# goroda/c3sc

Hardware: AMD Instinct MI355X
Metric: Bellman-sweep nodes/sec (7D car rank-10) (higher is better)
Workload: dtype f64

## Files before the change

c3sc_amd/csrc/c3sc_hip.hip:

```cpp
#include <hip/hip_runtime.h>

#include <algorithm>
#include <cmath>
#include <cstdio>
#include <cstdlib>
#include <cstring>
#include <string>
#include <vector>

#include "../../include/c3sc_hip.h"
#include "fiber_partition.hpp"
#include "kernel_chain_walk.hpp"
#include "kernel_common.hpp"
#include "kernel_rollout.hpp"
#include "kernel_rollout_ode.hpp"
#include "model_tables.hpp"
#include "registry.hpp"

namespace c3sc {

std::vector<KernelEntry> &kernel_registry()
{
    static std::vector<KernelEntry> reg;
    return reg;
}

__global__ void k_pad_core(const double *__restrict__ src, double *__restrict__ dst, int N, int r0, int r1, int RP,
                           int kind )
{
    const int per = (kind == 1) ? RP * RP : RP;
    const long total = (long)N * per;
    for (long e = (long)blockIdx.x * blockDim.x + threadIdx.x; e < total; e += (long)gridDim.x * blockDim.x) {
        const int j = (int)(e / per), w = (int)(e - (long)j * per);
        int a, b;
        if (kind == 0) { a = 0; b = w; }
        else if (kind == 2) { a = w; b = 0; }
        else { a = w % RP; b = w / RP; }
        double v = 0.0;
        if (a < r0 && b < r1) v = src[(size_t)j * r0 * r1 + a + (size_t)b * r0];
// ... 21 lines not shown
        const long total = (long)J.nodes[jb] * n2 * RP;
        for (long e = (long)blockIdx.x * blockDim.x + threadIdx.x; e < total; e += (long)gridDim.x * blockDim.x) {
            const long row = e / RP;
            const int c = (int)(e - row * RP), a = (int)(row / n2), b = (int)(row - (long)a * n2);
            const double *vec = left ? core + (size_t)a * RP : core2 + (size_t)b * RP;
            const double *mat = left ? core2 + (size_t)b * RP * RP + (size_t)c * RP : core + (size_t)a * RP * RP + c;
            const int ms = left ? 1 : RP;
            double t = 0.0;
            for (int s = 0; s < RP; s++) t = fma(vec[s], mat[(size_t)s * ms], t);
            img[e] = t;
        }
        return;
    }
    const long total = (long)J.nodes[jb] * stride;
    for (long e = (long)blockIdx.x * blockDim.x + threadIdx.x; e < total; e += (long)gridDim.x * blockDim.x) {
        const int j = (int)(e / stride), w = (int)(e - (long)j * stride);
        img[e] = (w < per) ? core[(size_t)j * per + w] : 0.0;
    }
}

struct Tab3Jobs {
    long tab2[2], core[2], dst[2];
    int n3[2], npairs[2];
};
__global__ void k_pair_tab3(double *__restrict__ arena, const Tab3Jobs J, int RP)
{
    const int sd = blockIdx.y;
    const bool left = sd == 0;
    const double *tab2 = arena + J.tab2[sd], *core = arena + J.core[sd];
    double *dst = arena + J.dst[sd];
    const long np = J.npairs[sd], total = (long)J.n3[sd] * np * RP;
    for (long e = (long)blockIdx.x * blockDim.x + threadIdx.x; e < total; e += (long)gridDim.x * blockDim.x) {
        const long row = e / RP;
        const int c = (int)(e - row * RP);
        const long i3 = row / np, pair = row - i3 * np;
        const double *vec = tab2 + pair * RP;
        const double *mat = left ? core + i3 * RP * RP + (long)c * RP : core + i3 * RP * RP + c;
        const int ms = left ? 1 : RP;
        double t = 0.0;
        for (int s = 0; s < RP; s++) t = fma(vec[s], mat[(long)s * ms], t);
        dst[e] = t;
    }
}

__global__ void k_quad_aux(const double *__restrict__ core, double *__restrict__ coreT, double *__restrict__ aop, int N, int RP)
{
    const int C = RP / 4, MB = (C + 3) / 4;
    const int per_t = RP * RP, per_a = 2 * MB * C * 64;
    const long total = (long)N * (per_t + per_a);
    for (long e = (long)blockIdx.x * blockDim.x + threadIdx.x; e < total; e += (long)gridDim.x * blockDim.x) {
        const int j = (int)(e / (per_t + per_a)), w = (int)(e - (long)j * (per_t + per_a));
// ... 753 lines not shown
        double *dst[MAXD];
        for (int m = 0; m < d; m++) dst[m] = buf.data() + (offs[(size_t)s * MAXD + m] - (long)c->static_doubles);
        pad_cores_host(d, c->ngrid, rps[s], ranks + (size_t)s * (d + 1), cores + (size_t)s * d, dst);
    }
    HIPCHK(c, hipSetDevice(c->device));
    if (c->hz_stack) HIPCHK(c, hipFree(c->hz_stack));
    c->hz_stack = nullptr;
    c->hz_nstack = 0;
    HIPCHK(c, hipMalloc((void **)&c->hz_stack, off * sizeof(double)));
    HIPCHK(c, hipMemcpy(c->hz_stack + c->static_doubles, buf.data(), buf.size() * sizeof(double), hipMemcpyHostToDevice));
    c->hz_stack_static = c->static_doubles;
    c->hz_rp.swap(rps);
    c->hz_core_off.swap(offs);
    c->hz_nstack = nstack;
    return C3SC_OK;
}

int c3sc_hip_upload_value_device(c3sc_hip_ctx *c, const size_t *ranks, const double *const *d_cores, void *stream)
{
    size_t cd = 0;
    int rc = prepare_value(c, ranks, &cd);
    if (rc != C3SC_OK) return rc;
    const int d = c->d, rp = c->rp;
    for (int m = 0; m < d; m++) {
        const int kind = (m == 0) ? 0 : (m == d - 1 ? 2 : 1);
        const long total = (long)c->ngrid[m] * (kind == 1 ? rp * rp : rp);
        const int grid = (int)std::min<long>((total + 255) / 256, 1024);
        hipLaunchKernelGGL(k_pad_core, dim3(grid), dim3(256), 0, (hipStream_t)stream, d_cores[m], c->arena + c->core_off[m],
                           c->ngrid[m], (int)ranks[m], (int)ranks[m + 1], rp, kind);
    }
    HIPCHK(c, hipGetLastError());
    rc = make_quad_aux(c, stream);
    if (rc != C3SC_OK) return rc;
    c->have_value = true;
    return C3SC_OK;
}

static int fill_args(c3sc_hip_ctx *c, int k, size_t F, KArgs &A, bool need_model)
{
    if (!c) return C3SC_ERR_ARG;
    if (c->d == 0 || !c->have_boundary || !c->have_value) return fail(c, C3SC_ERR_ARG, "launch: grid, boundary and value must be set");
    if (need_model && (!c->have_mca || c->model == 0 || c->ncand == 0))
        return fail(c, C3SC_ERR_ARG, "launch: mca, model and controls must be set");
    if (k < 0 || k >= c->d) return fail(c, C3SC_ERR_ARG, "launch: dim_vary out of range");
    HIPCHK(c, hipSetDevice(c->device));
    if (c->static_dirty) {
        if (static_layout(c) != c->static_doubles)
            return fail(c, C3SC_ERR_ARG, "launch: static data changed size after upload_value; upload the value again");
        int rc = upload_static(c);
        if (rc != C3SC_OK) return rc;
    }
    std::memset(&A, 0, sizeof(A));
    A.d = c->d;
// ... 52 lines not shown
    A.memo_keys = c->memo.keys; A.memo_vals = c->memo.vals; A.memo_capmask = c->memo.capmask; A.memo_epoch_bits = c->memo.epoch_bits;
    A.memo_shift = c->memo.shift; A.memo_counters = c->memo.counters; A.memo_mode = c->memo.mode;
    for (int m = 0; m < c->d; m++) A.memo_stride[m] = c->memo.stride[m];
    c->memo.applied = true;
}

static hipError_t ctx_launch(const c3sc_hip_ctx *c, const KernelEntry &e, const KArgs &A, LaunchIO io)
{
    io.form = c->switches;
    return launch_entry(e, A, io);
}

static int launch_one(c3sc_hip_ctx *c, const KernelEntry *e, const KArgs &A, const LaunchIO &io, const char *unsupported = nullptr)
{
    c->last_kernel = e->name;
    g_launches++;
    c->status_cache_valid = false;
    const hipError_t he = ctx_launch(c, *e, A, io);
    if (he == hipErrorNotSupported && unsupported) return fail(c, C3SC_ERR_UNSUPPORTED, unsupported);
    HIPCHK(c, he);
    return C3SC_OK;
}

constexpr long FIBER_PARTITION_MIN = 524288;
static long fiber_partition_min()
{
    const char *e = getenv("C3SC_FIBER_PARTITION");
    if (!e || !*e) return FIBER_PARTITION_MIN;
    const long v = atol(e);
    return v > 0 ? v : -1;
}

static long fiber_group_floor()
{
    const char *e = getenv("C3SC_FIBER_GROUP");
    if (!e || !*e) return FPART_MIN_PER_BIN;
    const long v = atol(e);
    return v > 0 ? v : -1;
}

static bool partitions(const KernelEntry *e, const KArgs &A)
{
    if (e->variant != C3SC_VARIANT_FIBER_PAIR || e->rtc || A.ncand > 64) return false;
    bool faces = false;
    for (int m = 0; m < A.d; m++) faces = faces || (m != A.k && A.bctype[m] == C3SC_ABSORB);
    const long fmin = fiber_partition_min();
    return faces && fmin >= 0 && A.F >= fmin && A.F <= 0x40000000L;
}

static bool runs_tab3(const c3sc_hip_ctx *c, const KernelEntry *e, const KArgs &A)
{
    if (!c->tab3L_off || fpp_table3_optout(A.d, e->rp, A.k) || !partitions(e, A)) return false;
    const char *env = getenv("C3SC_PAIR_TABLE3");
    return !(env && *env && atol(env) == 0);
}

static int ensure_tab3(c3sc_hip_ctx *c, hipStream_t st)
{
    if (!c->tab3_stale) {
        if (st != c->tab3_stream) HIPCHK(c, hipStreamWaitEvent(st, c->tab3_ev, 0));
        return C3SC_OK;
    }
    const int d = c->d, rp = c->rp;
    if (!c->tab3_ev) HIPCHK(c, hipEventCreateWithFlags(&c->tab3_ev, hipEventDisableTiming));
    Tab3Jobs J;
    J.tab2[0] = c->tabL_off; J.core[0] = c->core_off[2]; J.dst[0] = c->tab3L_off;
    J.n3[0] = c->ngrid[2]; J.npairs[0] = c->ngrid[0] * c->ngrid[1];
    J.tab2[1] = c->tabR_off; J.core[1] = c->core_off[d - 3]; J.dst[1] = c->tab3R_off;
    J.n3[1] = c->ngrid[d - 3]; J.npairs[1] = c->ngrid[d - 2] * c->ngrid[d - 1];
    const long total = std::max((long)J.n3[0] * J.npairs[0], (long)J.n3[1] * J.npairs[1]) * rp;
    hipLaunchKernelGGL(k_pair_tab3, dim3((unsigned)std::min<long>((total + 255) / 256, 4096), 2), dim3(256), 0, st, c->arena, J, rp);
    HIPCHK(c, hipGetLastError());
    HIPCHK(c, hipEventRecord(c->tab3_ev, st));
    c->tab3_stream = st;
    c->tab3_stale = false;
    return C3SC_OK;
}

static int partition_fibers(c3sc_hip_ctx *c, const KernelEntry *e, const KArgs &A, LaunchIO &io, int slot, int &launched)
{
    io.perm = nullptr;
    io.nlive = nullptr;
    launched = 0;
    if (!partitions(e, A)) return C3SC_OK;
    PartArgs P;
    P.d = A.d;
    P.k = A.k;
    P.F = A.F;
    for (int m = 0; m < MAXD; m++) { P.ngrid[m] = A.ngrid[m]; P.bctype[m] = A.bctype[m]; }
    fpart_plan(P, fpp_group_levels(A.d, e->rp, A.k), fiber_group_floor());
    const size_t need = fpart_bytes(A.F, P.nbins);
    if (need > c->part_bytes[slot]) {
        if (c->part[slot]) HIPCHK(c, hipFree(c->part[slot]));
        c->part[slot] = nullptr;
        c->part_bytes[slot] = 0;
        c->part_last[slot] = {};
        HIPCHK(c, hipMalloc(&c->part[slot], need));
        c->part_bytes[slot] = need;
    }
    const PartScratch ps = fpart_carve(c->part[slot], A.F, P.nbins);
    c->part_last[slot] = {ps.perm, ps.nlive, A.F, io.stream};
    HIPCHK(c, fpart_launch(P, io.idx, ps, io.stream));
    launched = 3;
    io.perm = ps.perm;
    io.nlive = ps.nlive;
    return C3SC_OK;
}

static int launch_bellman(c3sc_hip_ctx *c, int k, size_t F, const int32_t *d_idx, const int32_t *d_policy, double *d_out,
                          int32_t *d_uidx, int32_t *d_absorbed, void *stream, int part_slot = 0)
{
    KArgs A;
    int rc = fill_args(c, k, F, A, true);
    if (rc != C3SC_OK) return rc;
    int variant = c->variant;
    for (const FormRow &r : FORM_ROWS) {
        if (!(ctx_form(c) & r.bit)) continue;
        rc = check_form_model(c, "bellman_fibers", r.bit);
        if (rc != C3SC_OK) return rc;
        if (variant != C3SC_VARIANT_AUTO && variant != C3SC_VARIANT_FIBER_PER_WAVE)
            return fails(c, C3SC_ERR_UNSUPPORTED, "bellman_fibers: " + verb(r, "runs", "run") + " on the fiber-per-wave kernel only (the pair and quad variants have no " +
                                                      r.kind + " form)");
        variant = C3SC_VARIANT_FIBER_PER_WAVE;
    }
    if (F == 0) return C3SC_OK;
// ... 938 lines not shown
```

c3sc_amd/csrc/fiber_partition.hpp:

```cpp
#pragma once
#include <hip/hip_runtime.h>

#include "kernel_common.hpp"

namespace c3sc {

constexpr int FPART_THREADS = 256, FPART_PER_THREAD = 4, FPART_BLOCK = FPART_THREADS * FPART_PER_THREAD;
static_assert(FPART_BLOCK == 1024, "the scatter packs (bin, position in the block) into one word with 10 position bits");
constexpr int FPART_BIN_PER_THREAD = 8, FPART_MAX_BINS = FPART_THREADS * FPART_BIN_PER_THREAD;
constexpr long FPART_MIN_PER_BIN = 128;
constexpr int FPART_SCAN_BINS = 16;

struct PartArgs {
    int d, k;
    long F;
    int ngrid[MAXD];
    int bctype[MAXD];
    int kmaj = -1, kmin = -1;
    int nmin = 1;
    int nbins = 2;
};

constexpr void fpart_plan(PartArgs &P, KeyLevels kl, long floor)
{
    P.kmaj = P.kmin = -1;
    P.nmin = 1;
    P.nbins = 2;
    if (floor < 0 || kl.n < 1) return;
    const long nmaj = P.ngrid[kl.major];
    if (nmaj + 1 > FPART_MAX_BINS || P.F < floor * nmaj) return;
    P.kmaj = kl.major;
    P.nbins = (int)nmaj + 1;
    if (kl.n < 2) return;
    const long nkeys = nmaj * P.ngrid[kl.minor];
    if (nkeys + 1 > FPART_MAX_BINS || P.F < floor * nkeys) return;
    P.kmin = kl.minor;
    P.nmin = P.ngrid[kl.minor];
    P.nbins = (int)nkeys + 1;
}

struct PartScratch {
    int32_t *perm = nullptr;
    int32_t *counts = nullptr;
    int32_t *totals = nullptr;
    int32_t *nlive = nullptr;
    uint16_t *bins = nullptr;
};

__host__ __device__ constexpr size_t fpart_align(size_t b) { return (b + 255) & ~(size_t)255; }
constexpr long fpart_blocks(long F) { return (F + FPART_BLOCK - 1) / FPART_BLOCK; }
struct PartOffsets {
    size_t perm, counts, totals, nlive, bins, end;
};
constexpr PartOffsets fpart_offsets(long F, int nbins)
{
    PartOffsets o{};
    o.perm = 0;
    o.counts = o.perm + fpart_align((size_t)F * 4);
    o.totals = o.counts + fpart_align((size_t)fpart_blocks(F) * nbins * 4);
    o.nlive = o.totals + fpart_align((size_t)nbins * 4);
    o.bins = o.nlive + fpart_align(4);
    o.end = o.bins + fpart_align((size_t)F * 2);
    return o;
}
constexpr size_t fpart_bytes(long F, int nbins) { return fpart_offsets(F, nbins).end; }
inline PartScratch fpart_carve(void *base, long F, int nbins)
{
    const PartOffsets o = fpart_offsets(F, nbins);
    PartScratch s;
    char *p = (char *)base;
    s.perm = (int32_t *)(p + o.perm);
    s.counts = (int32_t *)(p + o.counts);
    s.totals = (int32_t *)(p + o.totals);
    s.nlive = (int32_t *)(p + o.nlive);
    s.bins = (uint16_t *)(p + o.bins);
    return s;
}

__device__ inline bool fiber_dead(const PartArgs &P, const int32_t *__restrict__ idx, long f)
{
    bool dead = false;
    for (int m = 0; m < P.d; m++) {
        if (m == P.k) continue;
        int lo, hi;
        dead = fixed_neighbors(idx[f * P.d + m], P.ngrid[m], P.bctype[m], lo, hi) || dead;
    }
    return dead;
}

__device__ inline int fpart_block_scan(int v, int &total)
{
    __shared__ int wsum[FPART_THREADS / 64];
    const int lane = threadIdx.x & 63, w = threadIdx.x >> 6;
    int inc = v;
#pragma unroll
    for (int o = 1; o < 64; o <<= 1) {
        const int t = __shfl_up(inc, o, 64);
        if (lane >= o) inc += t;
    }
    __syncthreads();
    if (lane == 63) wsum[w] = inc;
    __syncthreads();
    int before = 0;
    total = 0;
#pragma unroll
    for (int q = 0; q < FPART_THREADS / 64; q++) {
        if (q < w) before += wsum[q];
        total += wsum[q];
    }
    return before + inc - v;
}

__global__ void __launch_bounds__(FPART_THREADS) k_fpart_count(const PartArgs P, const int32_t *__restrict__ idx, uint16_t *__restrict__ bins,
                                                               int32_t *__restrict__ counts)
{
    __shared__ int hist[FPART_MAX_BINS];
    for (int b = threadIdx.x; b < P.nbins; b += FPART_THREADS) hist[b] = 0;
    __syncthreads();
    const long f0 = (long)blockIdx.x * FPART_BLOCK + threadIdx.x;
#pragma unroll
    for (int i = 0; i < FPART_PER_THREAD; i++) {
        const long f = f0 + (long)i * FPART_THREADS;
        if (f < P.F) {
            int bin = P.nbins - 1;
            if (!fiber_dead(P, idx, f)) {
                bin = P.kmaj >= 0 ? idx[f * P.d + P.kmaj] : 0;
                if (P.kmin >= 0) bin = bin * P.nmin + idx[f * P.d + P.kmin];
                bin = min(max(bin, 0), P.nbins - 2);
            }
            bins[f] = (uint16_t)bin;
            atomicAdd(&hist[bin], 1);
        }
    }
    __syncthreads();
    int32_t *row = counts + (size_t)blockIdx.x * P.nbins;
    for (int b = threadIdx.x; b < P.nbins; b += FPART_THREADS) row[b] = hist[b];
}

constexpr int FPART_SCAN_THREADS = 1024, FPART_SCAN_CHUNK = 8;
__global__ void __launch_bounds__(FPART_SCAN_THREADS) k_fpart_scan(int32_t *__restrict__ counts, long nblocks, int nbins, int32_t *__restrict__ totals)
{
    constexpr int NS = FPART_SCAN_THREADS / FPART_SCAN_BINS;
    __shared__ int part[NS][FPART_SCAN_BINS];
    const int c = threadIdx.x % FPART_SCAN_BINS, s = threadIdx.x / FPART_SCAN_BINS;
    const int bin = blockIdx.x * FPART_SCAN_BINS + c;
    const bool on = bin < nbins;
    const long per = (nblocks + NS - 1) / NS, b0 = s * per < nblocks ? s * per : nblocks, b1 = b0 + per < nblocks ? b0 + per : nblocks;
    int sum = 0;
    if (on)
        for (long b = b0; b < b1; b += FPART_SCAN_CHUNK) {
            int v[FPART_SCAN_CHUNK];
#pragma unroll
            for (int q = 0; q < FPART_SCAN_CHUNK; q++) v[q] = b + q < b1 ? counts[(size_t)(b + q) * nbins + bin] : 0;
#pragma unroll
            for (int q = 0; q < FPART_SCAN_CHUNK; q++) sum += v[q];
        }
    part[s][c] = sum;
    __syncthreads();
    int run = 0, total = 0;
    for (int q = 0; q < NS; q++) {
        const int v = part[q][c];
        if (q < s) run += v;
        total += v;
    }
    if (on) {
        for (long b = b0; b < b1; b += FPART_SCAN_CHUNK) {
            int v[FPART_SCAN_CHUNK];
#pragma unroll
            for (int q = 0; q < FPART_SCAN_CHUNK; q++) v[q] = b + q < b1 ? counts[(size_t)(b + q) * nbins + bin] : 0;
#pragma unroll
            for (int q = 0; q < FPART_SCAN_CHUNK; q++) {
                if (b + q < b1) counts[(size_t)(b + q) * nbins + bin] = run;
                run += v[q];
            }
        }
        if (s == 0) totals[bin] = total;
    }
}

__global__ void __launch_bounds__(FPART_THREADS) k_fpart_scatter(long F, int nbins, const uint16_t *__restrict__ bins, const int32_t *__restrict__ counts,
                                                                 const int32_t *__restrict__ totals, int32_t *__restrict__ nlive,
                                                                 int32_t *__restrict__ perm)
{
    __shared__ int base[FPART_MAX_BINS];
    __shared__ int start[FPART_MAX_BINS];
    __shared__ unsigned srt[FPART_BLOCK];
    const int tid = threadIdx.x;
    {
        int v[FPART_BIN_PER_THREAD], sum = 0;
#pragma unroll
        for (int i = 0; i < FPART_BIN_PER_THREAD; i++) {
            const int b = tid * FPART_BIN_PER_THREAD + i;
            v[i] = b < nbins ? totals[b] : 0;
            sum += v[i];
        }
        int total;
        int ex = fpart_block_scan(sum, total);
#pragma unroll
        for (int i = 0; i < FPART_BIN_PER_THREAD; i++) {
            base[tid * FPART_BIN_PER_THREAD + i] = ex;
            ex += v[i];
        }
    }
    const long fb = (long)blockIdx.x * FPART_BLOCK;
    if (nbins == 2) {
        if (blockIdx.x == 0 && tid == 0) *nlive = base[1];
        bool dead[FPART_PER_THREAD];
        int live = 0;
#pragma unroll
        for (int i = 0; i < FPART_PER_THREAD; i++) {
            const long f = fb + tid * FPART_PER_THREAD + i;
            dead[i] = f < F ? bins[f] != 0 : true;
            live += dead[i] ? 0 : 1;
        }
        int total;
        const int ex = fpart_block_scan(live, total);
        const int32_t *row = counts + (size_t)blockIdx.x * 2;
        long lpos = (long)row[0] + ex, dpos = (long)base[1] + row[1] + (tid * FPART_PER_THREAD - ex);
#pragma unroll
        for (int i = 0; i < FPART_PER_THREAD; i++) {
            const long f = fb + tid * FPART_PER_THREAD + i;
            if (f < F) {
                if (dead[i]) perm[dpos++] = (int32_t)f;
                else perm[lpos++] = (int32_t)f;
            }
        }
        return;
    }
#pragma unroll
    for (int i = 0; i < FPART_PER_THREAD; i++) {
        const int p = tid * FPART_PER_THREAD + i;
        srt[p] = fb + p < F ? ((unsigned)bins[fb + p] << 10) | (unsigned)p : 0xffffffffu;
    }
    for (int k = 2; k <= FPART_BLOCK; k <<= 1)
        for (int j = k >> 1; j > 0; j >>= 1) {
            __syncthreads();
#pragma unroll
            for (int e = tid; e < FPART_BLOCK / 2; e += FPART_THREADS) {
                const int lo = ((e & ~(j - 1)) << 1) | (e & (j - 1)), hi = lo | j;
                const unsigned a = srt[lo], b = srt[hi];
                const bool up = (lo & k) == 0;
                if ((a > b) == up) {
                    srt[lo] = b;
                    srt[hi] = a;
                }
            }
        }
    __syncthreads();
    if (blockIdx.x == 0 && tid == 0) *nlive = base[nbins - 1];
    unsigned w[FPART_PER_THREAD];
#pragma unroll
    for (int i = 0; i < FPART_PER_THREAD; i++) {
        const int s = tid * FPART_PER_THREAD + i;
        w[i] = srt[s];
        if (w[i] != 0xffffffffu && (s == 0 || (srt[s - 1] >> 10) != (w[i] >> 10))) start[w[i] >> 10] = s;
    }
    __syncthreads();
    const int32_t *row = counts + (size_t)blockIdx.x * nbins;
#pragma unroll
    for (int i = 0; i < FPART_PER_THREAD; i++) {
        if (w[i] != 0xffffffffu) {
            const int s = tid * FPART_PER_THREAD + i, bin = (int)(w[i] >> 10);
            perm[(long)base[bin] + row[bin] + (s - start[bin])] = (int32_t)(fb + (w[i] & 1023u));
        }
    }
}

inline hipError_t fpart_launch(const PartArgs &P, const int32_t *idx, const PartScratch &s, hipStream_t stream)
{
    const long nb = fpart_blocks(P.F);
    hipLaunchKernelGGL(k_fpart_count, dim3((unsigned)nb), dim3(FPART_THREADS), 0, stream, P, idx, s.bins, s.counts);
    hipLaunchKernelGGL(k_fpart_scan, dim3((unsigned)((P.nbins + FPART_SCAN_BINS - 1) / FPART_SCAN_BINS)), dim3(FPART_SCAN_THREADS), 0, stream, s.counts, nb,
                       P.nbins, s.totals);
    hipLaunchKernelGGL(k_fpart_scatter, dim3((unsigned)nb), dim3(FPART_THREADS), 0, stream, P.F, P.nbins, (const uint16_t *)s.bins,
                       (const int32_t *)s.counts, (const int32_t *)s.totals, s.nlive, s.perm);
    return hipGetLastError();
}

}
```

c3sc_amd/csrc/kernel_common.hpp:

```cpp
#pragma once
#ifdef __HIPCC_RTC__
#include "rtc_prelude.hpp"
#else
#include <type_traits>
#include <hip/hip_runtime.h>
#include <stdint.h>
#endif

#include "../../include/c3sc_hip.h"

#ifdef C3SC_STAMPS
#define C3SC_STAMPS_ON 1
#else
#define C3SC_STAMPS_ON 0
#endif

namespace c3sc {

constexpr int MAXD = C3SC_MAX_DIM;

struct KArgs {
    int d, k, N, ncand;
    long F;
    int ngrid[MAXD];
// ... 63 lines not shown
    if (nl > 0 && nr > 0) return {2, k - 1, k + 1};
    if (nl > 0) return {nl > 1 ? 2 : 1, k - 1, nl > 1 ? k - 2 : -1};
    if (nr > 0) return {nr > 1 ? 2 : 1, k + 1, nr > 1 ? k + 2 : -1};
    return {0, -1, -1};
}
#ifndef FPP_DIRECT_MAXD
#define FPP_DIRECT_MAXD 3
#endif
#ifndef FPP_EDGE_TABLES
#define FPP_EDGE_TABLES 1
#endif
#ifndef FPP_GROUP_FOLD
#define FPP_GROUP_FOLD 1
#endif
__host__ __device__ constexpr bool fpp_group_fold_optout(int d, int rp, int k) { return d == 7 && rp == 10 && k == 1; }
__host__ __device__ constexpr bool fpp_table3_registered(int d, int rp) { return FPP_EDGE_TABLES && d == 7 && rp == 10; }
__host__ __device__ constexpr bool pair_tab3_reserved(int d, const int *ngrid, int rp)
{
    return d >= 6 && fpp_table3_registered(d, rp) &&
           pair_tab3_doubles(ngrid[0], ngrid[1], ngrid[2], rp) * (long)sizeof(double) <= PAIR_TAB3_MAX_BYTES &&
           pair_tab3_doubles(ngrid[d - 3], ngrid[d - 2], ngrid[d - 1], rp) * (long)sizeof(double) <= PAIR_TAB3_MAX_BYTES;
}
__host__ __device__ constexpr bool fpp_table3_optout(int d, int rp, int k) { return d == 7 && rp == 10 && k >= 2; }
__host__ __device__ constexpr KeyLevels fpp_group_levels(int d, int rp, int k)
{
    const bool direct = d <= FPP_DIRECT_MAXD && rp <= 8;
    if (!FPP_GROUP_FOLD || direct || fpp_group_fold_optout(d, rp, k)) return {0, -1, -1};
    return fpp_key_levels(d, k, FPP_EDGE_TABLES && d >= 4);
}

__device__ inline int game_list_to_pair(const KArgs &A, int p)
{
    return A.game_order == C3SC_GAME_MAXMIN ? (p % A.game_gsz) * A.game_ngrp + p / A.game_gsz : p;
}
__device__ inline int game_pair_to_list(const KArgs &A, int i)
{
    return A.game_order == C3SC_GAME_MAXMIN ? (i % A.game_ngrp) * A.game_gsz + i / A.game_ngrp : i;
}

template <class M>
struct GameOf : M {
    static constexpr bool GAME = true;
};
template <class Model>
constexpr bool model_game()
{
// ... 1019 lines not shown
```

Baseline: 34.55 billion.

## Add rank-based fiber partition, batch core padding, trim unused table side

Replaces the per-block bitonic sort in the fiber partition scatter with a rank-based scheme that records each fiber's slot during counting, and pads count rows to cache-line strides. Core padding becomes a single batched launch across all dimensions. The pair table-3 precompute now builds only the sides that some sweep dimension reads, and the partition threshold is lowered so more sweeps use partitioning. This adds a new scratch array and more complex counting, and the lower threshold may apply partitioning overhead to smaller sweeps.

```diff
diff --git a/c3sc_amd/csrc/c3sc_hip.hip b/c3sc_amd/csrc/c3sc_hip.hip
--- a/c3sc_amd/csrc/c3sc_hip.hip
+++ b/c3sc_amd/csrc/c3sc_hip.hip
@@ -10,11 +10,13 @@
 
 #include "../../include/c3sc_hip.h"
 #include "fiber_partition.hpp"
+#include "fiber_partition_sort.hpp"
 #include "kernel_chain_walk.hpp"
 #include "kernel_common.hpp"
 #include "kernel_rollout.hpp"
 #include "kernel_rollout_ode.hpp"
 #include "model_tables.hpp"
+#include "pad_cores.hpp"
 #include "registry.hpp"
 
 namespace c3sc {
@@ -82,11 +84,12 @@
 struct Tab3Jobs {
     long tab2[2], core[2], dst[2];
     int n3[2], npairs[2];
+    int left[2];
 };
 __global__ void k_pair_tab3(double *__restrict__ arena, const Tab3Jobs J, int RP)
 {
     const int sd = blockIdx.y;
-    const bool left = sd == 0;
+    const bool left = J.left[sd] != 0;
     const double *tab2 = arena + J.tab2[sd], *core = arena + J.core[sd];
     double *dst = arena + J.dst[sd];
     const long np = J.npairs[sd], total = (long)J.n3[sd] * np * RP;
@@ -886,13 +889,18 @@
     int rc = prepare_value(c, ranks, &cd);
     if (rc != C3SC_OK) return rc;
     const int d = c->d, rp = c->rp;
+    PadJobs J{};
+    J.d = d;
+    long maxtotal = 1;
     for (int m = 0; m < d; m++) {
-        const int kind = (m == 0) ? 0 : (m == d - 1 ? 2 : 1);
-        const long total = (long)c->ngrid[m] * (kind == 1 ? rp * rp : rp);
-        const int grid = (int)std::min<long>((total + 255) / 256, 1024);
-        hipLaunchKernelGGL(k_pad_core, dim3(grid), dim3(256), 0, (hipStream_t)stream, d_cores[m], c->arena + c->core_off[m],
-                           c->ngrid[m], (int)ranks[m], (int)ranks[m + 1], rp, kind);
-    }
+        J.src[m] = d_cores[m];
+        J.dst[m] = c->core_off[m];
+        J.N[m] = c->ngrid[m];
+        J.r0[m] = (int)ranks[m];
+        J.r1[m] = (int)ranks[m + 1];
+        maxtotal = std::max(maxtotal, (long)c->ngrid[m] * ((m == 0 || m == d - 1) ? rp : rp * rp));
+    }
+    HIPCHK(c, pad_cores_launch(c->arena, J, rp, (unsigned)std::min<long>((maxtotal + 255) / 256, 1024), (hipStream_t)stream));
     HIPCHK(c, hipGetLastError());
     rc = make_quad_aux(c, stream);
     if (rc != C3SC_OK) return rc;
@@ -991,7 +999,7 @@
     return C3SC_OK;
 }
 
-constexpr long FIBER_PARTITION_MIN = 524288;
+constexpr long FIBER_PARTITION_MIN = 262144;
 static long fiber_partition_min()
 {
     const char *e = getenv("C3SC_FIBER_PARTITION");
@@ -1006,6 +1014,12 @@
     if (!e || !*e) return FPART_MIN_PER_BIN;
     const long v = atol(e);
     return v > 0 ? v : -1;
+}
+
+static bool fiber_rank()
+{
+    const char *e = getenv("C3SC_FIBER_RANK");
+    return !(e && *e && atol(e) == 0);
 }
 
 static bool partitions(const KernelEntry *e, const KArgs &A)
@@ -1032,14 +1046,28 @@
     }
     const int d = c->d, rp = c->rp;
     if (!c->tab3_ev) HIPCHK(c, hipEventCreateWithFlags(&c->tab3_ev, hipEventDisableTiming));
-    Tab3Jobs J;
-    J.tab2[0] = c->tabL_off; J.core[0] = c->core_off[2]; J.dst[0] = c->tab3L_off;
-    J.n3[0] = c->ngrid[2]; J.npairs[0] = c->ngrid[0] * c->ngrid[1];
-    J.tab2[1] = c->tabR_off; J.core[1] = c->core_off[d - 3]; J.dst[1] = c->tab3R_off;
-    J.n3[1] = c->ngrid[d - 3]; J.npairs[1] = c->ngrid[d - 2] * c->ngrid[d - 1];
-    const long total = std::max((long)J.n3[0] * J.npairs[0], (long)J.n3[1] * J.npairs[1]) * rp;
-    hipLaunchKernelGGL(k_pair_tab3, dim3((unsigned)std::min<long>((total + 255) / 256, 4096), 2), dim3(256), 0, st, c->arena, J, rp);
-    HIPCHK(c, hipGetLastError());
+    Tab3Jobs J{};
+    const Tab3Sides sides = fpp_table3_sides(d, rp);
+    int n = 0;
+    long total = 0;
+    if (sides.left) {
+        J.left[n] = 1;
+        J.tab2[n] = c->tabL_off; J.core[n] = c->core_off[2]; J.dst[n] = c->tab3L_off;
+        J.n3[n] = c->ngrid[2]; J.npairs[n] = c->ngrid[0] * c->ngrid[1];
+        total = std::max(total, (long)J.n3[n] * J.npairs[n] * rp);
+        n++;
+    }
+    if (sides.right) {
+        J.left[n] = 0;
+        J.tab2[n] = c->tabR_off; J.core[n] = c->core_off[d - 3]; J.dst[n] = c->tab3R_off;
+        J.n3[n] = c->ngrid[d - 3]; J.npairs[n] = c->ngrid[d - 2] * c->ngrid[d - 1];
+        total = std::max(total, (long)J.n3[n] * J.npairs[n] * rp);
+        n++;
+    }
+    if (n > 0) {
+        hipLaunchKernelGGL(k_pair_tab3, dim3((unsigned)std::min<long>((total + 255) / 256, 4096), (unsigned)n), dim3(256), 0, st, c->arena, J, rp);
+        HIPCHK(c, hipGetLastError());
+    }
     HIPCHK(c, hipEventRecord(c->tab3_ev, st));
     c->tab3_stream = st;
     c->tab3_stale = false;
@@ -1069,7 +1097,7 @@
     }
     const PartScratch ps = fpart_carve(c->part[slot], A.F, P.nbins);
     c->part_last[slot] = {ps.perm, ps.nlive, A.F, io.stream};
-    HIPCHK(c, fpart_launch(P, io.idx, ps, io.stream));
+    HIPCHK(c, fiber_rank() ? fpart_launch(P, io.idx, ps, io.stream) : fpart_launch_sorting(P, io.idx, ps, io.stream));
     launched = 3;
     io.perm = ps.perm;
     io.nlive = ps.nlive;
diff --git a/c3sc_amd/csrc/fiber_partition.hpp b/c3sc_amd/csrc/fiber_partition.hpp
--- a/c3sc_amd/csrc/fiber_partition.hpp
+++ b/c3sc_amd/csrc/fiber_partition.hpp
@@ -45,22 +45,26 @@
     int32_t *totals = nullptr;
     int32_t *nlive = nullptr;
     uint16_t *bins = nullptr;
+    uint16_t *rank = nullptr;
 };
 
 __host__ __device__ constexpr size_t fpart_align(size_t b) { return (b + 255) & ~(size_t)255; }
 constexpr long fpart_blocks(long F) { return (F + FPART_BLOCK - 1) / FPART_BLOCK; }
+constexpr int FPART_LINE_INTS = 32;
+__host__ __device__ constexpr int fpart_stride(int nbins) { return (nbins + FPART_LINE_INTS - 1) / FPART_LINE_INTS * FPART_LINE_INTS; }
 struct PartOffsets {
-    size_t perm, counts, totals, nlive, bins, end;
+    size_t perm, counts, totals, nlive, bins, rank, end;
 };
 constexpr PartOffsets fpart_offsets(long F, int nbins)
 {
     PartOffsets o{};
     o.perm = 0;
     o.counts = o.perm + fpart_align((size_t)F * 4);
-    o.totals = o.counts + fpart_align((size_t)fpart_blocks(F) * nbins * 4);
+    o.totals = o.counts + fpart_align((size_t)fpart_blocks(F) * fpart_stride(nbins) * 4);
     o.nlive = o.totals + fpart_align((size_t)nbins * 4);
     o.bins = o.nlive + fpart_align(4);
-    o.end = o.bins + fpart_align((size_t)F * 2);
+    o.rank = o.bins + fpart_align((size_t)F * 2);
+    o.end = o.rank + fpart_align((size_t)F * 2);
     return o;
 }
 constexpr size_t fpart_bytes(long F, int nbins) { return fpart_offsets(F, nbins).end; }
@@ -74,6 +78,7 @@
     s.totals = (int32_t *)(p + o.totals);
     s.nlive = (int32_t *)(p + o.nlive);
     s.bins = (uint16_t *)(p + o.bins);
+    s.rank = (uint16_t *)(p + o.rank);
     return s;
 }
 
@@ -111,170 +116,7 @@
     return before + inc - v;
 }
 
-__global__ void __launch_bounds__(FPART_THREADS) k_fpart_count(const PartArgs P, const int32_t *__restrict__ idx, uint16_t *__restrict__ bins,
-                                                               int32_t *__restrict__ counts)
-{
-    __shared__ int hist[FPART_MAX_BINS];
-    for (int b = threadIdx.x; b < P.nbins; b += FPART_THREADS) hist[b] = 0;
-    __syncthreads();
-    const long f0 = (long)blockIdx.x * FPART_BLOCK + threadIdx.x;
-#pragma unroll
-    for (int i = 0; i < FPART_PER_THREAD; i++) {
-        const long f = f0 + (long)i * FPART_THREADS;
-        if (f < P.F) {
-            int bin = P.nbins - 1;
-            if (!fiber_dead(P, idx, f)) {
-                bin = P.kmaj >= 0 ? idx[f * P.d + P.kmaj] : 0;
-                if (P.kmin >= 0) bin = bin * P.nmin + idx[f * P.d + P.kmin];
-                bin = min(max(bin, 0), P.nbins - 2);
-            }
-            bins[f] = (uint16_t)bin;
-            atomicAdd(&hist[bin], 1);
-        }
-    }
-    __syncthreads();
-    int32_t *row = counts + (size_t)blockIdx.x * P.nbins;
-    for (int b = threadIdx.x; b < P.nbins; b += FPART_THREADS) row[b] = hist[b];
-}
-
-constexpr int FPART_SCAN_THREADS = 1024, FPART_SCAN_CHUNK = 8;
-__global__ void __launch_bounds__(FPART_SCAN_THREADS) k_fpart_scan(int32_t *__restrict__ counts, long nblocks, int nbins, int32_t *__restrict__ totals)
-{
-    constexpr int NS = FPART_SCAN_THREADS / FPART_SCAN_BINS;
-    __shared__ int part[NS][FPART_SCAN_BINS];
-    const int c = threadIdx.x % FPART_SCAN_BINS, s = threadIdx.x / FPART_SCAN_BINS;
-    const int bin = blockIdx.x * FPART_SCAN_BINS + c;
-    const bool on = bin < nbins;
-    const long per = (nblocks + NS - 1) / NS, b0 = s * per < nblocks ? s * per : nblocks, b1 = b0 + per < nblocks ? b0 + per : nblocks;
-    int sum = 0;
-    if (on)
-        for (long b = b0; b < b1; b += FPART_SCAN_CHUNK) {
-            int v[FPART_SCAN_CHUNK];
-#pragma unroll
-            for (int q = 0; q < FPART_SCAN_CHUNK; q++) v[q] = b + q < b1 ? counts[(size_t)(b + q) * nbins + bin] : 0;
-#pragma unroll
-            for (int q = 0; q < FPART_SCAN_CHUNK; q++) sum += v[q];
-        }
-    part[s][c] = sum;
-    __syncthreads();
-    int run = 0, total = 0;
-    for (int q = 0; q < NS; q++) {
-        const int v = part[q][c];
-        if (q < s) run += v;
-        total += v;
-    }
-    if (on) {
-        for (long b = b0; b < b1; b += FPART_SCAN_CHUNK) {
-            int v[FPART_SCAN_CHUNK];
-#pragma unroll
-            for (int q = 0; q < FPART_SCAN_CHUNK; q++) v[q] = b + q < b1 ? counts[(size_t)(b + q) * nbins + bin] : 0;
-#pragma unroll
-            for (int q = 0; q < FPART_SCAN_CHUNK; q++) {
-                if (b + q < b1) counts[(size_t)(b + q) * nbins + bin] = run;
-                run += v[q];
-            }
-        }
-        if (s == 0) totals[bin] = total;
-    }
-}
-
-__global__ void __launch_bounds__(FPART_THREADS) k_fpart_scatter(long F, int nbins, const uint16_t *__restrict__ bins, const int32_t *__restrict__ counts,
-                                                                 const int32_t *__restrict__ totals, int32_t *__restrict__ nlive,
-                                                                 int32_t *__restrict__ perm)
-{
-    __shared__ int base[FPART_MAX_BINS];
-    __shared__ int start[FPART_MAX_BINS];
-    __shared__ unsigned srt[FPART_BLOCK];
-    const int tid = threadIdx.x;
-    {
-        int v[FPART_BIN_PER_THREAD], sum = 0;
-#pragma unroll
-        for (int i = 0; i < FPART_BIN_PER_THREAD; i++) {
-            const int b = tid * FPART_BIN_PER_THREAD + i;
-            v[i] = b < nbins ? totals[b] : 0;
-            sum += v[i];
-        }
-        int total;
-        int ex = fpart_block_scan(sum, total);
-#pragma unroll
-        for (int i = 0; i < FPART_BIN_PER_THREAD; i++) {
-            base[tid * FPART_BIN_PER_THREAD + i] = ex;
-            ex += v[i];
-        }
-    }
-    const long fb = (long)blockIdx.x * FPART_BLOCK;
-    if (nbins == 2) {
-        if (blockIdx.x == 0 && tid == 0) *nlive = base[1];
-        bool dead[FPART_PER_THREAD];
-        int live = 0;
-#pragma unroll
-        for (int i = 0; i < FPART_PER_THREAD; i++) {
-            const long f = fb + tid * FPART_PER_THREAD + i;
-            dead[i] = f < F ? bins[f] != 0 : true;
-            live += dead[i] ? 0 : 1;
-        }
-        int total;
-        const int ex = fpart_block_scan(live, total);
-        const int32_t *row = counts + (size_t)blockIdx.x * 2;
-        long lpos = (long)row[0] + ex, dpos = (long)base[1] + row[1] + (tid * FPART_PER_THREAD - ex);
-#pragma unroll
-        for (int i = 0; i < FPART_PER_THREAD; i++) {
-            const long f = fb + tid * FPART_PER_THREAD + i;
-            if (f < F) {
-                if (dead[i]) perm[dpos++] = (int32_t)f;
-                else perm[lpos++] = (int32_t)f;
-            }
-        }
-        return;
-    }
-#pragma unroll
-    for (int i = 0; i < FPART_PER_THREAD; i++) {
-        const int p = tid * FPART_PER_THREAD + i;
-        srt[p] = fb + p < F ? ((unsigned)bins[fb + p] << 10) | (unsigned)p : 0xffffffffu;
-    }
-    for (int k = 2; k <= FPART_BLOCK; k <<= 1)
-        for (int j = k >> 1; j > 0; j >>= 1) {
-            __syncthreads();
-#pragma unroll
-            for (int e = tid; e < FPART_BLOCK / 2; e += FPART_THREADS) {
-                const int lo = ((e & ~(j - 1)) << 1) | (e & (j - 1)), hi = lo | j;
-                const unsigned a = srt[lo], b = srt[hi];
-                const bool up = (lo & k) == 0;
-                if ((a > b) == up) {
-                    srt[lo] = b;
-                    srt[hi] = a;
-                }
-            }
-        }
-    __syncthreads();
-    if (blockIdx.x == 0 && tid == 0) *nlive = base[nbins - 1];
-    unsigned w[FPART_PER_THREAD];
-#pragma unroll
-    for (int i = 0; i < FPART_PER_THREAD; i++) {
-        const int s = tid * FPART_PER_THREAD + i;
-        w[i] = srt[s];
-        if (w[i] != 0xffffffffu && (s == 0 || (srt[s - 1] >> 10) != (w[i] >> 10))) start[w[i] >> 10] = s;
-    }
-    __syncthreads();
-    const int32_t *row = counts + (size_t)blockIdx.x * nbins;
-#pragma unroll
-    for (int i = 0; i < FPART_PER_THREAD; i++) {
-        if (w[i] != 0xffffffffu) {
-            const int s = tid * FPART_PER_THREAD + i, bin = (int)(w[i] >> 10);
-            perm[(long)base[bin] + row[bin] + (s - start[bin])] = (int32_t)(fb + (w[i] & 1023u));
-        }
-    }
-}
-
-inline hipError_t fpart_launch(const PartArgs &P, const int32_t *idx, const PartScratch &s, hipStream_t stream)
-{
-    const long nb = fpart_blocks(P.F);
-    hipLaunchKernelGGL(k_fpart_count, dim3((unsigned)nb), dim3(FPART_THREADS), 0, stream, P, idx, s.bins, s.counts);
-    hipLaunchKernelGGL(k_fpart_scan, dim3((unsigned)((P.nbins + FPART_SCAN_BINS - 1) / FPART_SCAN_BINS)), dim3(FPART_SCAN_THREADS), 0, stream, s.counts, nb,
-                       P.nbins, s.totals);
-    hipLaunchKernelGGL(k_fpart_scatter, dim3((unsigned)nb), dim3(FPART_THREADS), 0, stream, P.F, P.nbins, (const uint16_t *)s.bins,
-                       (const int32_t *)s.counts, (const int32_t *)s.totals, s.nlive, s.perm);
-    return hipGetLastError();
-}
+hipError_t fpart_launch_sorting(const PartArgs &P, const int32_t *idx, const PartScratch &s, hipStream_t stream);
+hipError_t fpart_launch(const PartArgs &P, const int32_t *idx, const PartScratch &s, hipStream_t stream);
 
 }
diff --git a/c3sc_amd/csrc/fiber_partition_rank.hpp b/c3sc_amd/csrc/fiber_partition_rank.hpp
--- /dev/null
+++ b/c3sc_amd/csrc/fiber_partition_rank.hpp
@@ -0,0 +1,252 @@
+#pragma once
+#include "fiber_partition.hpp"
+
+namespace c3sc {
+
+constexpr int FPART_RANK_SORT_MIN = 64;
+
+__global__ void __launch_bounds__(FPART_THREADS) k_fpart_rank_count(const PartArgs P, const int32_t *__restrict__ idx, uint16_t *__restrict__ bins,
+                                                               uint16_t *__restrict__ rank, int32_t *__restrict__ counts, int sort_min)
+{
+    __shared__ int hist[FPART_MAX_BINS];
+    __shared__ int start[FPART_MAX_BINS];
+    __shared__ unsigned list[FPART_BLOCK];
+    __shared__ int ndead[FPART_PER_THREAD][FPART_THREADS / 64];
+    const int tid = threadIdx.x, lane = tid & 63, wv = tid >> 6;
+    for (int b = tid; b < P.nbins; b += FPART_THREADS) hist[b] = 0;
+    __syncthreads();
+    const long fb = (long)blockIdx.x * FPART_BLOCK;
+    const int deadbin = P.nbins - 1;
+    int bin[FPART_PER_THREAD], slot[FPART_PER_THREAD], dbefore[FPART_PER_THREAD];
+#pragma unroll
+    for (int i = 0; i < FPART_PER_THREAD; i++) {
+        const long f = fb + i * FPART_THREADS + tid;
+        bin[i] = -1;
+        slot[i] = 0;
+        if (f < P.F) {
+            int b = deadbin;
+            if (!fiber_dead(P, idx, f)) {
+                b = P.kmaj >= 0 ? idx[f * P.d + P.kmaj] : 0;
+                if (P.kmin >= 0) b = b * P.nmin + idx[f * P.d + P.kmin];
+                b = min(max(b, 0), P.nbins - 2);
+            }
+            bin[i] = b;
+            bins[f] = (uint16_t)b;
+            slot[i] = atomicAdd(&hist[b], 1);
+        }
+        const unsigned long long dm = __ballot(bin[i] == deadbin);
+        dbefore[i] = __popcll(dm & ((1ull << lane) - 1ull));
+        if (lane == 0) ndead[i][wv] = __popcll(dm);
+    }
+    __syncthreads();
+    int32_t *row = counts + (size_t)blockIdx.x * fpart_stride(P.nbins);
+    for (int b = tid; b < P.nbins; b += FPART_THREADS) row[b] = hist[b];
+    if (P.nbins == 2) return;
+#pragma unroll
+    for (int i = 0; i < FPART_PER_THREAD; i++) {
+        int r = dbefore[i];
+#pragma unroll
+        for (int q = 0; q < FPART_PER_THREAD * (FPART_THREADS / 64); q++)
+            if (q < i * (FPART_THREADS / 64) + wv) r += ndead[q / (FPART_THREADS / 64)][q % (FPART_THREADS / 64)];
+        if (bin[i] == deadbin) rank[fb + i * FPART_THREADS + tid] = (uint16_t)r;
+    }
+    int v[FPART_BIN_PER_THREAD], sum = 0, most = 0;
+#pragma unroll
+    for (int i = 0; i < FPART_BIN_PER_THREAD; i++) {
+        const int b = tid * FPART_BIN_PER_THREAD + i;
+        v[i] = b < deadbin ? hist[b] : 0;
+        sum += v[i];
+        most = max(most, v[i]);
+    }
+    if (!__syncthreads_or(most >= sort_min)) {
+        int total;
+        int ex = fpart_block_scan(sum, total);
+#pragma unroll
+        for (int i = 0; i < FPART_BIN_PER_THREAD; i++) {
+            start[tid * FPART_BIN_PER_THREAD + i] = ex;
+            ex += v[i];
+        }
+        __syncthreads();
+        int s0[FPART_PER_THREAD], n[FPART_PER_THREAD], r[FPART_PER_THREAD], nmost = 0;
+#pragma unroll
+        for (int i = 0; i < FPART_PER_THREAD; i++) {
+            const bool live = bin[i] >= 0 && bin[i] != deadbin;
+            s0[i] = live ? start[bin[i]] : 0;
+            n[i] = live ? hist[bin[i]] : 0;
+            r[i] = 0;
+            nmost = max(nmost, n[i]);
+            if (live) list[s0[i] + slot[i]] = (unsigned)(i * FPART_THREADS + tid);
+        }
+        __syncthreads();
+        for (int j = 0; j < nmost; j++) {
+#pragma unroll
+            for (int i = 0; i < FPART_PER_THREAD; i++)
+                if (j < n[i]) r[i] += list[s0[i] + j] < (unsigned)(i * FPART_THREADS + tid) ? 1 : 0;
+        }
+#pragma unroll
+        for (int i = 0; i < FPART_PER_THREAD; i++)
+            if (n[i] > 0) rank[fb + i * FPART_THREADS + tid] = (uint16_t)r[i];
+        return;
+    }
+#pragma unroll
+    for (int i = 0; i < FPART_PER_THREAD; i++) {
+        const int p = i * FPART_THREADS + tid;
+        list[p] = bin[i] >= 0 && bin[i] != deadbin ? ((unsigned)bin[i] << 10) | (unsigned)p : 0xffffffffu;
+    }
+    for (int k = 2; k <= FPART_BLOCK; k <<= 1)
+        for (int j = k >> 1; j > 0; j >>= 1) {
+            __syncthreads();
+#pragma unroll
+            for (int e = tid; e < FPART_BLOCK / 2; e += FPART_THREADS) {
+                const int lo = ((e & ~(j - 1)) << 1) | (e & (j - 1)), hi = lo | j;
+                const unsigned a = list[lo], b = list[hi];
+                const bool up = (lo & k) == 0;
+                if ((a > b) == up) {
+                    list[lo] = b;
+                    list[hi] = a;
+                }
+            }
+        }
+    __syncthreads();
+    unsigned w[FPART_PER_THREAD];
+#pragma unroll
+    for (int i = 0; i < FPART_PER_THREAD; i++) {
+        const int s = tid * FPART_PER_THREAD + i;
+        w[i] = list[s];
+        if (w[i] != 0xffffffffu && (s == 0 || (list[s - 1] >> 10) != (w[i] >> 10))) start[w[i] >> 10] = s;
+    }
+    __syncthreads();
+#pragma unroll
+    for (int i = 0; i < FPART_PER_THREAD; i++)
+        if (w[i] != 0xffffffffu) rank[fb + (w[i] & 1023u)] = (uint16_t)(tid * FPART_PER_THREAD + i - start[w[i] >> 10]);
+}
+
+constexpr int FPART_RSCAN_BINS = FPART_LINE_INTS;
+constexpr int FPART_RSCAN_THREADS = 1024, FPART_RSCAN_CHUNK = 8, FPART_RSCAN_SEGS = FPART_RSCAN_THREADS / FPART_RSCAN_BINS, FPART_RSCAN_KEEP = 32;
+__global__ void __launch_bounds__(FPART_RSCAN_THREADS) k_fpart_rank_scan(int32_t *__restrict__ counts, long nblocks, int nbins, int32_t *__restrict__ totals)
+{
+    constexpr int NS = FPART_RSCAN_SEGS;
+    __shared__ int part[NS][FPART_RSCAN_BINS];
+    const int c = threadIdx.x % FPART_RSCAN_BINS, s = threadIdx.x / FPART_RSCAN_BINS;
+    const int bin = blockIdx.x * FPART_RSCAN_BINS + c;
+    const bool on = bin < nbins;
+    const int stride = fpart_stride(nbins);
+    const long per = (nblocks + NS - 1) / NS, b0 = s * per < nblocks ? s * per : nblocks, b1 = b0 + per < nblocks ? b0 + per : nblocks;
+    const bool keep = per <= FPART_RSCAN_KEEP;
+    int kept[FPART_RSCAN_KEEP];
+    int sum = 0;
+    if (on && keep) {
+#pragma unroll
+        for (int q = 0; q < FPART_RSCAN_KEEP; q++) {
+            const long b = b0 + q < b1 ? b0 + q : nblocks - 1;
+            kept[q] = counts[(size_t)b * stride + bin];
+        }
+#pragma unroll
+        for (int q = 0; q < FPART_RSCAN_KEEP; q++) {
+            kept[q] = b0 + q < b1 ? kept[q] : 0;
+            sum += kept[q];
+        }
+    } else if (on) {
+        for (long b = b0; b < b1; b += FPART_RSCAN_CHUNK) {
+            int v[FPART_RSCAN_CHUNK];
+#pragma unroll
+            for (int q = 0; q < FPART_RSCAN_CHUNK; q++) v[q] = b + q < b1 ? counts[(size_t)(b + q) * stride + bin] : 0;
+#pragma unroll
+            for (int q = 0; q < FPART_RSCAN_CHUNK; q++) sum += v[q];
+        }
+    }
+    part[s][c] = sum;
+    __syncthreads();
+    int run = 0, total = 0;
+    for (int q = 0; q < NS; q++) {
+        const int v = part[q][c];
+        if (q < s) run += v;
+        total += v;
+    }
+    if (!on) return;
+    if (s == 0) totals[bin] = total;
+    if (keep) {
+#pragma unroll
+        for (int q = 0; q < FPART_RSCAN_KEEP; q++) {
+            if (b0 + q < b1) counts[(size_t)(b0 + q) * stride + bin] = run;
+            run += kept[q];
+        }
+        return;
+    }
+    for (long b = b0; b < b1; b += FPART_RSCAN_CHUNK) {
+        int v[FPART_RSCAN_CHUNK];
+#pragma unroll
+        for (int q = 0; q < FPART_RSCAN_CHUNK; q++) v[q] = b + q < b1 ? counts[(size_t)(b + q) * stride + bin] : 0;
+#pragma unroll
+        for (int q = 0; q < FPART_RSCAN_CHUNK; q++) {
+            if (b + q < b1) counts[(size_t)(b + q) * stride + bin] = run;
+            run += v[q];
+        }
+    }
+}
+
+__global__ void __launch_bounds__(FPART_THREADS) k_fpart_rank_scatter(long F, int nbins, const uint16_t *__restrict__ bins, const uint16_t *__restrict__ rank,
+                                                                 const int32_t *__restrict__ counts, const int32_t *__restrict__ totals,
+                                                                 int32_t *__restrict__ nlive, int32_t *__restrict__ perm)
+{
+    __shared__ int base[FPART_MAX_BINS];
+    const int tid = threadIdx.x;
+    const long blk = (long)(blockIdx.x % 8) * (gridDim.x / 8) + blockIdx.x / 8;
+    if (blk * FPART_BLOCK >= F) return;
+    {
+        int v[FPART_BIN_PER_THREAD], sum = 0;
+#pragma unroll
+        for (int i = 0; i < FPART_BIN_PER_THREAD; i++) {
+            const int b = tid * FPART_BIN_PER_THREAD + i;
+            v[i] = b < nbins ? totals[b] : 0;
+            sum += v[i];
+        }
+        int total;
+        int ex = fpart_block_scan(sum, total);
+#pragma unroll
+        for (int i = 0; i < FPART_BIN_PER_THREAD; i++) {
+            base[tid * FPART_BIN_PER_THREAD + i] = ex;
+            ex += v[i];
+        }
+    }
+    const long fb = blk * FPART_BLOCK;
+    if (nbins == 2) {
+        if (blk == 0 && tid == 0) *nlive = base[1];
+        bool dead[FPART_PER_THREAD];
+        int live = 0;
+#pragma unroll
+        for (int i = 0; i < FPART_PER_THREAD; i++) {
+            const long f = fb + tid * FPART_PER_THREAD + i;
+            dead[i] = f < F ? bins[f] != 0 : true;
+            live += dead[i] ? 0 : 1;
+        }
+        int total;
+        const int ex = fpart_block_scan(live, total);
+        const int32_t *row = counts + (size_t)blk * fpart_stride(2);
+        long lpos = (long)row[0] + ex, dpos = (long)base[1] + row[1] + (tid * FPART_PER_THREAD - ex);
+#pragma unroll
+        for (int i = 0; i < FPART_PER_THREAD; i++) {
+            const long f = fb + tid * FPART_PER_THREAD + i;
+            if (f < F) {
+                if (dead[i]) perm[dpos++] = (int32_t)f;
+                else perm[lpos++] = (int32_t)f;
+            }
+        }
+        return;
+    }
+    __syncthreads();
+    if (blk == 0 && tid == 0) *nlive = base[nbins - 1];
+    const int32_t *row = counts + (size_t)blk * fpart_stride(nbins);
+#pragma unroll
+    for (int i = 0; i < FPART_PER_THREAD; i++) {
+        const long f = fb + i * FPART_THREADS + tid;
+        if (f < F) {
+            const int bin = bins[f];
+            const long at = (long)base[bin] + row[bin] + rank[f];
+            if (at >= 0 && at < F) perm[at] = (int32_t)f;
+
+        }
+    }
+}
+
+}
diff --git a/c3sc_amd/csrc/fiber_partition_sort.hpp b/c3sc_amd/csrc/fiber_partition_sort.hpp
--- /dev/null
+++ b/c3sc_amd/csrc/fiber_partition_sort.hpp
@@ -0,0 +1,172 @@
+#pragma once
+#include "fiber_partition.hpp"
+
+namespace c3sc {
+
+__global__ void __launch_bounds__(FPART_THREADS) k_fpart_count(const PartArgs P, const int32_t *__restrict__ idx, uint16_t *__restrict__ bins,
+                                                               int32_t *__restrict__ counts)
+{
+    __shared__ int hist[FPART_MAX_BINS];
+    for (int b = threadIdx.x; b < P.nbins; b += FPART_THREADS) hist[b] = 0;
+    __syncthreads();
+    const long f0 = (long)blockIdx.x * FPART_BLOCK + threadIdx.x;
+#pragma unroll
+    for (int i = 0; i < FPART_PER_THREAD; i++) {
+        const long f = f0 + (long)i * FPART_THREADS;
+        if (f < P.F) {
+            int bin = P.nbins - 1;
+            if (!fiber_dead(P, idx, f)) {
+                bin = P.kmaj >= 0 ? idx[f * P.d + P.kmaj] : 0;
+                if (P.kmin >= 0) bin = bin * P.nmin + idx[f * P.d + P.kmin];
+                bin = min(max(bin, 0), P.nbins - 2);
+            }
+            bins[f] = (uint16_t)bin;
+            atomicAdd(&hist[bin], 1);
+        }
+    }
+    __syncthreads();
+    int32_t *row = counts + (size_t)blockIdx.x * P.nbins;
+    for (int b = threadIdx.x; b < P.nbins; b += FPART_THREADS) row[b] = hist[b];
+}
+
+constexpr int FPART_SCAN_THREADS = 1024, FPART_SCAN_CHUNK = 8;
+__global__ void __launch_bounds__(FPART_SCAN_THREADS) k_fpart_scan(int32_t *__restrict__ counts, long nblocks, int nbins, int32_t *__restrict__ totals)
+{
+    constexpr int NS = FPART_SCAN_THREADS / FPART_SCAN_BINS;
+    __shared__ int part[NS][FPART_SCAN_BINS];
+    const int c = threadIdx.x % FPART_SCAN_BINS, s = threadIdx.x / FPART_SCAN_BINS;
+    const int bin = blockIdx.x * FPART_SCAN_BINS + c;
+    const bool on = bin < nbins;
+    const long per = (nblocks + NS - 1) / NS, b0 = s * per < nblocks ? s * per : nblocks, b1 = b0 + per < nblocks ? b0 + per : nblocks;
+    int sum = 0;
+    if (on)
+        for (long b = b0; b < b1; b += FPART_SCAN_CHUNK) {
+            int v[FPART_SCAN_CHUNK];
+#pragma unroll
+            for (int q = 0; q < FPART_SCAN_CHUNK; q++) v[q] = b + q < b1 ? counts[(size_t)(b + q) * nbins + bin] : 0;
+#pragma unroll
+            for (int q = 0; q < FPART_SCAN_CHUNK; q++) sum += v[q];
+        }
+    part[s][c] = sum;
+    __syncthreads();
+    int run = 0, total = 0;
+    for (int q = 0; q < NS; q++) {
+        const int v = part[q][c];
+        if (q < s) run += v;
+        total += v;
+    }
+    if (on) {
+        for (long b = b0; b < b1; b += FPART_SCAN_CHUNK) {
+            int v[FPART_SCAN_CHUNK];
+#pragma unroll
+            for (int q = 0; q < FPART_SCAN_CHUNK; q++) v[q] = b + q < b1 ? counts[(size_t)(b + q) * nbins + bin] : 0;
+#pragma unroll
+            for (int q = 0; q < FPART_SCAN_CHUNK; q++) {
+                if (b + q < b1) counts[(size_t)(b + q) * nbins + bin] = run;
+                run += v[q];
+            }
+        }
+        if (s == 0) totals[bin] = total;
+    }
+}
+
+__global__ void __launch_bounds__(FPART_THREADS) k_fpart_scatter(long F, int nbins, const uint16_t *__restrict__ bins, const int32_t *__restrict__ counts,
+                                                                 const int32_t *__restrict__ totals, int32_t *__restrict__ nlive,
+                                                                 int32_t *__restrict__ perm)
+{
+    __shared__ int base[FPART_MAX_BINS];
+    __shared__ int start[FPART_MAX_BINS];
+    __shared__ unsigned srt[FPART_BLOCK];
+    const int tid = threadIdx.x;
+    {
+        int v[FPART_BIN_PER_THREAD], sum = 0;
+#pragma unroll
+        for (int i = 0; i < FPART_BIN_PER_THREAD; i++) {
+            const int b = tid * FPART_BIN_PER_THREAD + i;
+            v[i] = b < nbins ? totals[b] : 0;
+            sum += v[i];
+        }
+        int total;
+        int ex = fpart_block_scan(sum, total);
+#pragma unroll
+        for (int i = 0; i < FPART_BIN_PER_THREAD; i++) {
+            base[tid * FPART_BIN_PER_THREAD + i] = ex;
+            ex += v[i];
+        }
+    }
+    const long fb = (long)blockIdx.x * FPART_BLOCK;
+    if (nbins == 2) {
+        if (blockIdx.x == 0 && tid == 0) *nlive = base[1];
+        bool dead[FPART_PER_THREAD];
+        int live = 0;
+#pragma unroll
+        for (int i = 0; i < FPART_PER_THREAD; i++) {
+            const long f = fb + tid * FPART_PER_THREAD + i;
+            dead[i] = f < F ? bins[f] != 0 : true;
+            live += dead[i] ? 0 : 1;
+        }
+        int total;
+        const int ex = fpart_block_scan(live, total);
+        const int32_t *row = counts + (size_t)blockIdx.x * 2;
+        long lpos = (long)row[0] + ex, dpos = (long)base[1] + row[1] + (tid * FPART_PER_THREAD - ex);
+#pragma unroll
+        for (int i = 0; i < FPART_PER_THREAD; i++) {
+            const long f = fb + tid * FPART_PER_THREAD + i;
+            if (f < F) {
+                if (dead[i]) perm[dpos++] = (int32_t)f;
+                else perm[lpos++] = (int32_t)f;
+            }
+        }
+        return;
+    }
+#pragma unroll
+    for (int i = 0; i < FPART_PER_THREAD; i++) {
+        const int p = tid * FPART_PER_THREAD + i;
+        srt[p] = fb + p < F ? ((unsigned)bins[fb + p] << 10) | (unsigned)p : 0xffffffffu;
+    }
+    for (int k = 2; k <= FPART_BLOCK; k <<= 1)
+        for (int j = k >> 1; j > 0; j >>= 1) {
+            __syncthreads();
+#pragma unroll
+            for (int e = tid; e < FPART_BLOCK / 2; e += FPART_THREADS) {
+                const int lo = ((e & ~(j - 1)) << 1) | (e & (j - 1)), hi = lo | j;
+                const unsigned a = srt[lo], b = srt[hi];
+                const bool up = (lo & k) == 0;
+                if ((a > b) == up) {
+                    srt[lo] = b;
+                    srt[hi] = a;
+                }
+            }
+        }
+    __syncthreads();
+    if (blockIdx.x == 0 && tid == 0) *nlive = base[nbins - 1];
+    unsigned w[FPART_PER_THREAD];
+#pragma unroll
+    for (int i = 0; i < FPART_PER_THREAD; i++) {
+        const int s = tid * FPART_PER_THREAD + i;
+        w[i] = srt[s];
+        if (w[i] != 0xffffffffu && (s == 0 || (srt[s - 1] >> 10) != (w[i] >> 10))) start[w[i] >> 10] = s;
+    }
+    __syncthreads();
+    const int32_t *row = counts + (size_t)blockIdx.x * nbins;
+#pragma unroll
+    for (int i = 0; i < FPART_PER_THREAD; i++) {
+        if (w[i] != 0xffffffffu) {
+            const int s = tid * FPART_PER_THREAD + i, bin = (int)(w[i] >> 10);
+            perm[(long)base[bin] + row[bin] + (s - start[bin])] = (int32_t)(fb + (w[i] & 1023u));
+        }
+    }
+}
+
+hipError_t fpart_launch_sorting(const PartArgs &P, const int32_t *idx, const PartScratch &s, hipStream_t stream)
+{
+    const long nb = fpart_blocks(P.F);
+    hipLaunchKernelGGL(k_fpart_count, dim3((unsigned)nb), dim3(FPART_THREADS), 0, stream, P, idx, s.bins, s.counts);
+    hipLaunchKernelGGL(k_fpart_scan, dim3((unsigned)((P.nbins + FPART_SCAN_BINS - 1) / FPART_SCAN_BINS)), dim3(FPART_SCAN_THREADS), 0, stream, s.counts, nb,
+                       P.nbins, s.totals);
+    hipLaunchKernelGGL(k_fpart_scatter, dim3((unsigned)nb), dim3(FPART_THREADS), 0, stream, P.F, P.nbins, (const uint16_t *)s.bins,
+                       (const int32_t *)s.counts, (const int32_t *)s.totals, s.nlive, s.perm);
+    return hipGetLastError();
+}
+
+}
diff --git a/c3sc_amd/csrc/kernel_common.hpp b/c3sc_amd/csrc/kernel_common.hpp
--- a/c3sc_amd/csrc/kernel_common.hpp
+++ b/c3sc_amd/csrc/kernel_common.hpp
@@ -109,6 +109,20 @@
            pair_tab3_doubles(ngrid[d - 3], ngrid[d - 2], ngrid[d - 1], rp) * (long)sizeof(double) <= PAIR_TAB3_MAX_BYTES;
 }
 __host__ __device__ constexpr bool fpp_table3_optout(int d, int rp, int k) { return d == 7 && rp == 10 && k >= 2; }
+struct Tab3Sides {
+    bool left, right;
+};
+__host__ __device__ constexpr Tab3Sides fpp_table3_sides(int d, int rp)
+{
+    Tab3Sides s{false, false};
+    for (int k = 0; k < d; k++) {
+        if (fpp_table3_optout(d, rp, k)) continue;
+        s.left = s.left || k >= 3;
+        s.right = s.right || k <= d - 4;
+    }
+    return s;
+}
+static_assert(!fpp_table3_sides(7, 10).left && fpp_table3_sides(7, 10).right, "car7d at rank 10: K = 0, 1 read the right table alone");
 __host__ __device__ constexpr KeyLevels fpp_group_levels(int d, int rp, int k)
 {
     const bool direct = d <= FPP_DIRECT_MAXD && rp <= 8;
diff --git a/c3sc_amd/csrc/pad_cores.hpp b/c3sc_amd/csrc/pad_cores.hpp
--- /dev/null
+++ b/c3sc_amd/csrc/pad_cores.hpp
@@ -0,0 +1,16 @@
+#pragma once
+#include <hip/hip_runtime.h>
+
+#include "kernel_common.hpp"
+
+namespace c3sc {
+
+struct PadJobs {
+    const double *src[MAXD];
+    long dst[MAXD];
+    int N[MAXD], r0[MAXD], r1[MAXD];
+    int d;
+};
+hipError_t pad_cores_launch(double *arena, const PadJobs &J, int rp, unsigned gridx, hipStream_t stream);
+
+}
diff --git a/c3sc_amd/csrc/prepass.hip b/c3sc_amd/csrc/prepass.hip
--- /dev/null
+++ b/c3sc_amd/csrc/prepass.hip
@@ -0,0 +1,44 @@
+#include "fiber_partition_rank.hpp"
+#include "pad_cores.hpp"
+
+namespace c3sc {
+
+hipError_t fpart_launch(const PartArgs &P, const int32_t *idx, const PartScratch &s, hipStream_t stream)
+{
+    const long nb = fpart_blocks(P.F);
+    hipLaunchKernelGGL(k_fpart_rank_count, dim3((unsigned)nb), dim3(FPART_THREADS), 0, stream, P, idx, s.bins, s.rank, s.counts, FPART_RANK_SORT_MIN);
+    hipLaunchKernelGGL(k_fpart_rank_scan, dim3((unsigned)((P.nbins + FPART_RSCAN_BINS - 1) / FPART_RSCAN_BINS)), dim3(FPART_RSCAN_THREADS), 0, stream,
+                       s.counts, nb, P.nbins, s.totals);
+    hipLaunchKernelGGL(k_fpart_rank_scatter, dim3((unsigned)((nb + 7) / 8 * 8)), dim3(FPART_THREADS), 0, stream, P.F, P.nbins, (const uint16_t *)s.bins,
+                       (const uint16_t *)s.rank, (const int32_t *)s.counts, (const int32_t *)s.totals, s.nlive, s.perm);
+    return hipGetLastError();
+}
+
+__global__ void k_pad_cores(double *__restrict__ arena, const PadJobs J, int RP)
+{
+    const int m = blockIdx.y;
+    const int kind = (m == 0) ? 0 : (m == J.d - 1 ? 2 : 1);
+    const double *__restrict__ src = J.src[m];
+    double *__restrict__ dst = arena + J.dst[m];
+    const int N = J.N[m], r0 = J.r0[m], r1 = J.r1[m];
+    const int per = (kind == 1) ? RP * RP : RP;
+    const long total = (long)N * per;
+    for (long e = (long)blockIdx.x * blockDim.x + threadIdx.x; e < total; e += (long)gridDim.x * blockDim.x) {
+        const int j = (int)(e / per), w = (int)(e - (long)j * per);
+        int a, b;
+        if (kind == 0) { a = 0; b = w; }
+        else if (kind == 2) { a = w; b = 0; }
+        else { a = w % RP; b = w / RP; }
+        double v = 0.0;
+        if (a < r0 && b < r1) v = src[(size_t)j * r0 * r1 + a + (size_t)b * r0];
+        dst[e] = v;
+    }
+}
+
+hipError_t pad_cores_launch(double *arena, const PadJobs &J, int rp, unsigned gridx, hipStream_t stream)
+{
+    hipLaunchKernelGGL(k_pad_cores, dim3(gridx, (unsigned)J.d), dim3(256), 0, stream, arena, J, rp);
+    return hipGetLastError();
+}
+
+}
```

Result: faster. 34.97 billion, median of 6 (+1.2%).
